# ambicuity/Distributed-LLM-Training-and-Inference-System

Hardware: AMD Instinct MI355X
Metric: tokens/sec (node) GPT-7B train (higher is better)
Workload: dtype bf16; 1 GPU; model=gpt-7b, global_batch=16, seq_len=2048, parallelism=dp1, micro_batch=16, grad_accum=1, activation_checkpoint=none, layout=planner

## Files before the change

llmctl/config/knobs.py:

```python

from __future__ import annotations

import contextlib
import dataclasses
import os
from dataclasses import dataclass, fields
from typing import Any, Dict, Iterator, Optional

ENV = "LLMCTL_KNOBS"


@dataclass(frozen=True)
class PerfKnobs:
    gemm64: bool = True
    gemm64_config: int = 304
    fwd64: str = "auto"
    dgrad64: str = "fused"
    wgrad_kernel: bool = True
    swiglu_bwd: str = "side"
    dgrad_transpose: bool = True
    wt_side_stream: bool = True
    fused_fwd: bool = False
    rope_inplace: bool = True
    fused_rope_attn: bool = True
    moe_pad: bool = True
    overlap_optimizer: bool = False
    gemm_tuning: bool = True
    fa_split: int = -1
    fa_prio: int = 1
    fa_nw: int = 4
    dkv: int = 2
    dkv_nwg: int = 0
    async_tp: bool = True
    async_tp_save_full: bool = False
    cp_zigzag: bool = True
    decode_fused: bool = True
    decode_splits: int = 0
    decode_v3: int = 1
    skinny_gemm: str = "auto"
    prefill_swiglu: bool = True
    prefill_fa: bool = True
    prefill_norm_fold: bool = True
    mixed_steps: bool = True
    custom_ar: bool = True
    tp_graphs: bool = True
    async_decode: bool = True
    tp_fused_decode: bool = True

    def as_dict(self) -> Dict[str, Any]:
        return dataclasses.asdict(self)


NATIVE = ("fa_split", "fa_prio", "fa_nw", "dkv", "dkv_nwg", "decode_splits", "decode_v3")
_FIELDS = {f.name: f for f in fields(PerfKnobs)}


def _coerce(name: str, value: Any) -> Any:
    if name not in _FIELDS:
        raise KeyError(f"unknown performance knob {name!r} (known: {', '.join(sorted(_FIELDS))})")
    typ = _FIELDS[name].type
    if typ in ("bool", bool):
        if isinstance(value, str):
            v = value.strip().lower()
            if v not in ("1", "0", "true", "false", "on", "off", "yes", "no"):
                raise ValueError(f"knob {name}: expected a boolean, got {value!r}")
            return v in ("1", "true", "on", "yes")
        return bool(value)
    if typ in ("int", int):
        return int(value)
    return str(value)


def parse_env(spec: Optional[str]) -> Dict[str, Any]:
    out: Dict[str, Any] = {}
    for part in (spec or "").split(","):
        part = part.strip()
        if not part:
            continue
        if "=" not in part:
            raise ValueError(f"{ENV}: expected name=value, got {part!r}")
        k, v = part.split("=", 1)
        out[k.strip()] = _coerce(k.strip(), v.strip())
    return out


_RETIRED_ENV = ("LLMCTL_SIDE_DGRAD", "LLMCTL_DECODE_ATTN_QKV", "LLMCTL_GEMM64_CONFIG", "LLMCTL_SKINNY")
_warned: set = set()


def _warn_retired_env() -> None:
    import warnings

    names = [f"LLMCTL_{n.upper()}" for n in _FIELDS] + list(_RETIRED_ENV)
    for n in names:
        if n in os.environ and n not in _warned:
            _warned.add(n)
            warnings.warn(f"{n} is no longer read (performance switches are knobs now): set "
                          f"{ENV}=\"{n[7:].lower()}=<value>\" or the [perf] config table instead", stacklevel=3)


def resolve(overrides: Optional[Dict[str, Any]] = None, env: bool = True) -> PerfKnobs:
    _warn_retired_env()
    kw = {k: _coerce(k, v) for k, v in (overrides or {}).items()}
    if env:
        kw.update(parse_env(os.environ.get(ENV)))
    return PerfKnobs(**kw)


_ACTIVE: PerfKnobs = resolve()


def knobs() -> PerfKnobs:
    return _ACTIVE


def push_native(k: Optional[PerfKnobs] = None) -> bool:
    k = k or _ACTIVE
    try:
        from llmctl.ops import _lib

        if not _lib.loaded():
            return False
        import torch

        for name in NATIVE:
            torch.ops.llmctl.set_knob(name, int(getattr(k, name)))
        return True
    except Exception:
        return False


def apply(k: PerfKnobs) -> PerfKnobs:
    global _ACTIVE
    _ACTIVE = k
    push_native(k)
    return k


def use(k: PerfKnobs) -> PerfKnobs:
    if k is not _ACTIVE:
        apply(k)
    return k


def with_env(k: PerfKnobs) -> PerfKnobs:
    env = parse_env(os.environ.get(ENV))
    return dataclasses.replace(k, **env) if env else k


def configure(overrides: Optional[Dict[str, Any]] = None) -> PerfKnobs:
    return apply(resolve(overrides))


@contextlib.contextmanager
def override(**kw: Any) -> Iterator[PerfKnobs]:
    old = _ACTIVE
    new = dataclasses.replace(old, **{k: _coerce(k, v) for k, v in kw.items()})
    apply(new)
    try:
        yield new
    finally:
        apply(old)
```

llmctl/ops/csrc/flash_attn_bwd.hip:

```cpp
#include <cstdlib>
#include <map>
#include <mutex>

#include "attn_common.h"

namespace llmctl {
using namespace attn;
namespace {

constexpr float LOG2E = 1.4426950408889634f;
constexpr int KV_KB = 128;
constexpr int KV_QT = 64;
#ifndef LLMCTL_DKV_NBUF
#define LLMCTL_DKV_NBUF 2
#endif
constexpr int KV_NBUF = LLMCTL_DKV_NBUF;
static_assert(KV_NBUF >= 2 && KV_NBUF <= 4, "dK/dV ring depth 2-4");
constexpr int DQ_QB = 128;
constexpr int DQ_KB = 64;

struct BwdArgs {
  const unsigned short *q, *k, *v, *dout;
  const float* lse;
  const float* delta;
// ... 701 lines not shown
  const int nkb = a.S / KV_KB;
  const int BH = a.B * a.Hkv;
  const bool per_xcd = BH % 8 == 0;
  const int xq = per_xcd ? (int)(blockIdx.x & 7) : 0;
  const int n_items = (per_xcd ? BH / 8 : BH) * nkb;
  const int bh_base = per_xcd ? xq * (BH / 8) : 0;
  const int group = a.Hq / a.Hkv;
  auto pop = [&]() __attribute__((always_inline)) -> int {
    const int j = __hip_atomic_fetch_add(wq + xq, 1, __ATOMIC_RELAXED, __HIP_MEMORY_SCOPE_AGENT);
    return j < n_items ? j : -1;
  };
  if (tid == 0) {
    const int i0 = pop();
    item_w[1] = i0;
    item_w[2] = i0 >= 0 ? pop() : -1;
  }
  __syncthreads();
  int cur = __builtin_amdgcn_readfirstlane(item_w[1]);
  int nxt = __builtin_amdgcn_readfirstlane(item_w[2]);
  if (cur < 0) return;

  const unsigned lds0 = lds_addr(smem);
  unsigned vq[NP], vd[NP];
#pragma unroll
  for (int i = 0; i < NP; ++i) {
    const int byte = (i * 4 + wave) * 1024 + lane * 16;
    const int row = byte / ROWB;
    const int lch = ((byte % ROWB) >> 4) ^ swz_tr<HD>(row);
    vq[i] = (unsigned)((row * a.q_ss + lch * 8) * 2);
    vd[i] = (unsigned)((row * a.do_ss + lch * 8) * 2);
  }
  const float* rc_src = a.rck_w + (wave == 1 ? a.rc_n : 0);
  const unsigned rc_off =
      (unsigned)((32 * (lane >> 5) + 8 * ((lane >> 2) & 3) + 4 * ((lane >> 4) & 1) + (lane & 3)) * 4);

  int iss = cur, iq0 = 0, iq_start = 0, ig = 0;
  const unsigned short *qh = nullptr, *dh = nullptr;
  const float* rh = nullptr;
  bool look_pending = false;
  int n_switch = 0;
  int pend0 = -1, pend1 = -1, npend = 0;
  auto iss_begin = [&](int item) __attribute__((always_inline)) {
    const int bh = bh_base + item / nkb, kb = item % nkb;
    const int bb = bh / a.Hkv, hkk = bh % a.Hkv;
    iq_start = kb * KV_KB;
    iq0 = iq_start;
    ig = 0;
    qh = a.q + bb * a.q_sb + (long)(hkk * group) * a.q_sh;
    dh = a.dout + bb * a.do_sb + (long)(hkk * group) * a.do_sh;
    rh = rc_src + ((long)bb * a.Hq + hkk * group) * a.S;
  };
  iss_begin(cur);
  auto issue = [&](auto slot_c) __attribute__((always_inline)) {
    constexpr int SLC = decltype(slot_c)::value;
    i32x4_t rq = buf_rsrc(qh + (long)iq0 * a.q_ss, (unsigned)(((KV_QT - 1) * a.q_ss + HD) * 2));
    i32x4_t rd = buf_rsrc(dh + (long)iq0 * a.do_ss, (unsigned)(((KV_QT - 1) * a.do_ss + HD) * 2));
    i32x4_t rr = buf_rsrc(rh + iq0, (unsigned)(KV_QT * 4));
    asm volatile("s_nop 4" : "+s"(rq), "+s"(rd), "+s"(rr));
    const unsigned slot = lds0 + (unsigned)(SLC * BUF_B);
#pragma unroll
    for (int i = 0; i < NP; ++i) {
      buf_dma16(rq, vq[i], slot + (i * 4 + wave) * 1024);
      buf_dma16(rd, vd[i], slot + TILE_B + (i * 4 + wave) * 1024);
    }
    buf_dma4(rr, rc_off, slot + 2 * TILE_B + wave * RC_B);
    iq0 += KV_QT;
    if (iq0 >= a.S) {
      if (++ig < group) {
        iq0 = iq_start;
        qh += a.q_sh;
        dh += a.do_sh;
        rh += a.S;
      } else {
        iss = nxt;
        if (iss >= 0) {
          iss_begin(iss);
          if (tid == 0) item_w[3 + (n_switch & 1)] = pop();
          look_pending = true;
          ++n_switch;
        }
        if (npend == 0) pend0 = iss;
        else pend1 = iss;
        ++npend;
      }
    }
  };

  bf16x8_t kf[NKS], vf[NKS];
  auto load_kv = [&](int item) __attribute__((always_inline)) {
    const int bh = bh_base + item / nkb, kb = item % nkb;
    const int bb = bh / a.Hkv, hkk = bh % a.Hkv;
    const int key = kb * KV_KB + wave * 32 + r;
    const unsigned short* Kp = a.k + bb * a.k_sb + hkk * a.k_sh + (long)key * a.k_ss + 8 * hh;
    const unsigned short* Vp = a.v + bb * a.v_sb + hkk * a.v_sh + (long)key * a.v_ss + 8 * hh;
#pragma unroll
    for (int ks = 0; ks < NKS; ++ks) {
      asm volatile("global_load_dwordx4 %0, %1, off" : "+a"(kf[ks]) : "v"(Kp + 16 * ks) : "memory");
      asm volatile("global_load_dwordx4 %0, %1, off" : "+a"(vf[ks]) : "v"(Vp + 16 * ks) : "memory");
    }
  };

  issue(std::integral_constant<int, 0>{});
  load_kv(cur);
  asm volatile("s_waitcnt vmcnt(0)"
               : "+a"(kf[0]), "+a"(kf[1]), "+a"(kf[2]), "+a"(kf[3]), "+a"(kf[4]), "+a"(kf[5]), "+a"(kf[6]),
                 "+a"(kf[7]), "+a"(vf[0]), "+a"(vf[1]), "+a"(vf[2]), "+a"(vf[3]), "+a"(vf[4]), "+a"(vf[5]),
                 "+a"(vf[6]), "+a"(vf[7])
               :
               : "memory");
  __builtin_amdgcn_s_barrier();
  issue(std::integral_constant<int, 1>{});
  f32x16 dk[NDB], dv[NDB];
#pragma unroll
  for (int d = 0; d < NDB; ++d) {
    const bf16x8_t z = {};
    asm volatile("s_nop 2\n\tv_mfma_f32_32x32x16_bf16 %0, %1, %1, 0" : "=a"(dk[d]) : "v"(z));
    asm volatile("v_mfma_f32_32x32x16_bf16 %0, %1, %1, 0" : "=a"(dv[d]) : "v"(z));
  }
  const float c = a.scale_log2;

  int n_done = 0;
  auto stamp = [&](int k) __attribute__((always_inline)) {
    if constexpr (STAMP) {
      if (tid == 0 && n_done < 64)
        a.stamps[(blockIdx.x * 64 + n_done) * 4 + k] = k == 3 ? (unsigned long long)cur : __builtin_amdgcn_s_memrealtime();
    }
  };
  for (;;) {
    stamp(0);
    stamp(3);
    const int bh = bh_base + cur / nkb, kb = cur % nkb;
    const int b = bh / a.Hkv, hk = bh % a.Hkv;
    const int k0 = kb * KV_KB;
    const int wkey0 = k0 + wave * 32;
    const int my_key = wkey0 + r;
    const int ntiles = group * ((a.S - k0) / KV_QT);
    int q0 = k0;
    auto apply_mask = [&](f32x16& s, int h) __attribute__((always_inline)) {
#pragma unroll
      for (int gq = 0; gq < 4; ++gq) {
        const int row0 = q0 + 32 * h + 8 * gq + 4 * hh;
#pragma unroll
        for (int j = 0; j < 4; ++j) s[4 * gq + j] = my_key <= row0 + j ? s[4 * gq + j] : -INFINITY;
      }
    };
    auto tile = [&](auto slot_c) __attribute__((always_inline)) {
      constexpr int SL = decltype(slot_c)::value;
      const bool live = !(wkey0 > q0 + KV_QT - 1);
      if (!live) return;
      const unsigned char* Qs = smem + SL * BUF_B;
      const unsigned char* Ds = Qs + TILE_B;
      const float* lse_s = reinterpret_cast<const float*>(Ds + TILE_B);
      const float* del_s = lse_s + KV_QT;
      const bool need_mask = wkey0 + 31 > q0;
      f32x16 s0 = *reinterpret_cast<const f32x16*>(lse_s + 16 * hh);
      f32x16 p0 = *reinterpret_cast<const f32x16*>(del_s + 16 * hh);
      bf16x8_t qa[NKS], da[NKS];
#pragma unroll
      for (int ks = 0; ks < NKS; ++ks) {
        qa[ks] = lds_read_b128(Qs, tr_off<HD>(r, 2 * ks + hh));
        da[ks] = lds_read_b128(Ds, tr_off<HD>(r, 2 * ks + hh));
      }
      f32x16 s1 = *reinterpret_cast<const f32x16*>(lse_s + 32 + 16 * hh);
      f32x16 p1 = *reinterpret_cast<const f32x16*>(del_s + 32 + 16 * hh);
      bf16x8_t qb[NKS], db[NKS];
#pragma unroll
      for (int ks = 0; ks < NKS; ++ks) {
        mfma_v(s0, qa[ks], kf[ks]);
        qb[ks] = lds_read_b128(Qs, tr_off<HD>(32 + r, 2 * ks + hh));
        mfma_v(p0, da[ks], vf[ks]);
        db[ks] = lds_read_b128(Ds, tr_off<HD>(32 + r, 2 * ks + hh));
      }
      if (need_mask) apply_mask(s0, 0);
      unsigned pw0[8], dw0[8];
      bf16x8_t td[2][NDB], tq[2][NDB];
#pragma unroll
      for (int ks = 0; ks < NKS; ++ks) {
        x_step(s1, p1, qb[ks], kf[ks], db[ks], vf[ks], s0[2 * ks], s0[2 * ks + 1], p0[2 * ks], p0[2 * ks + 1], c,
               pw0[ks], dw0[ks]);
        const int st = ks >> 2, d = ks & 3;
        td[st][d] = tr_frag<HD>(Ds, 16 * st, d * 32, lane);
        tq[st][d] = tr_frag<HD>(Qs, 16 * st, d * 32, lane);
      }
      if (need_mask) apply_mask(s1, 1);
      unsigned pw1[8], dw1[8];
      bf16x8_t cd[2][NDB], cq[2][NDB];
#pragma unroll
      for (int st = 0; st < 2; ++st) {
        const bf16x8_t pb = words8(pw0[4 * st], pw0[4 * st + 1], pw0[4 * st + 2], pw0[4 * st + 3]);
        const bf16x8_t sb = words8(dw0[4 * st], dw0[4 * st + 1], dw0[4 * st + 2], dw0[4 * st + 3]);
#pragma unroll
        for (int d = 0; d < NDB; ++d) {
          const int i = 4 * st + d;
          y_step(dv[d], dk[d], td[st][d], tq[st][d], pb, sb, s1[2 * i], s1[2 * i + 1], p1[2 * i], p1[2 * i + 1], c,
                 pw1[i], dw1[i]);
          cd[st][d] = tr_frag<HD>(Ds, 32 + 16 * st, d * 32, lane);
          cq[st][d] = tr_frag<HD>(Qs, 32 + 16 * st, d * 32, lane);
        }
      }
#pragma unroll
      for (int st = 0; st < 2; ++st) {
        const bf16x8_t pb = words8(pw1[4 * st], pw1[4 * st + 1], pw1[4 * st + 2], pw1[4 * st + 3]);
        const bf16x8_t sb = words8(dw1[4 * st], dw1[4 * st + 1], dw1[4 * st + 2], dw1[4 * st + 3]);
#pragma unroll
        for (int d = 0; d < NDB; ++d) z_step(dv[d], dk[d], cd[st][d], cq[st][d], pb, sb);
      }
    };
    auto advance = [&](auto slot_c) __attribute__((always_inline)) {
      constexpr int SL = decltype(slot_c)::value;
      asm volatile("s_waitcnt lgkmcnt(0)" ::: "memory");
      vm_wait_n<0>();
      __builtin_amdgcn_s_barrier();
      if (look_pending) {
        nxt = __builtin_amdgcn_readfirstlane(item_w[3 + ((n_switch - 1) & 1)]);
        look_pending = false;
      }
      if (iss >= 0) issue(std::integral_constant<int, SL>{});
      q0 += KV_QT;
      if (q0 >= a.S) q0 = k0;
    };
    for (int t = 0; t < ntiles; t += 2) {
      tile(std::integral_constant<int, 0>{});
      advance(std::integral_constant<int, 0>{});
      tile(std::integral_constant<int, 1>{});
      advance(std::integral_constant<int, 1>{});
    }
    stamp(1);
    {
      const long tok = (long)b * a.S + my_key;
      unsigned short* dkp = a.dk + tok * a.dk_st + (long)hk * HD;
      unsigned short* dvp = a.dv + tok * a.dv_st + (long)hk * HD;
      const bool rope = a.cos_t != nullptr;
      f32x4 cs[NDB / 2][4], sn[NDB / 2][4];
      if (rope) {
        const long p = a.rope_pos ? (long)a.rope_pos[tok] : tok % a.rope_S;
        const float* cr = a.cos_t + p * (HD / 2);
        const float* sr = a.sin_t + p * (HD / 2);
#pragma unroll
        for (int d = 0; d < NDB / 2; ++d)
#pragma unroll
          for (int g = 0; g < 4; ++g) {
            const int col = d * 32 + 8 * g + 4 * hh;
            cs[d][g] = *reinterpret_cast<const f32x4*>(cr + col);
            sn[d][g] = *reinterpret_cast<const f32x4*>(sr + col);
          }
      }
#pragma unroll
      for (int d = 0; d < NDB; ++d) asm volatile("s_nop 7\n\ts_nop 7" : "+a"(dk[d]), "+a"(dv[d]));
      auto st8 = [&](unsigned short* p, const float* x, float mul) __attribute__((always_inline)) {
        s2_t w;
        w[0] = (unsigned)f2bf(x[0] * mul) | ((unsigned)f2bf(x[1] * mul) << 16);
        w[1] = (unsigned)f2bf(x[2] * mul) | ((unsigned)f2bf(x[3] * mul) << 16);
        asm volatile("global_store_dwordx2 %0, %1, off" ::"v"(p), "v"(w) : "memory");
      };
#pragma unroll
      for (int d = 0; d < NDB / 2; ++d) {
        const f32x16 x1 = acc_copy(dk[d]), x2 = acc_copy(dk[d + NDB / 2]);
        acc_zero(dk[d]);
        acc_zero(dk[d + NDB / 2]);
#pragma unroll
        for (int g = 0; g < 4; ++g) {
          const int col = d * 32 + 8 * g + 4 * hh;
          float lo[4], hi[4];
#pragma unroll
          for (int j = 0; j < 4; ++j) {
            const float c1 = rope ? cs[d][g][j] : 1.f, s1 = rope ? sn[d][g][j] : 0.f;
            lo[j] = x1[4 * g + j] * c1 + x2[4 * g + j] * s1;
            hi[j] = x2[4 * g + j] * c1 - x1[4 * g + j] * s1;
          }
          st8(dkp + col, lo, a.scale);
          st8(dkp + col + HD / 2, hi, a.scale);
        }
      }
#pragma unroll
      for (int d = 0; d < NDB; ++d) {
        const f32x16 x = acc_copy(dv[d]);
        acc_zero(dv[d]);
#pragma unroll
        for (int g = 0; g < 4; ++g) {
          float y[4];
#pragma unroll
          for (int j = 0; j < 4; ++j) y[j] = x[4 * g + j];
          st8(dvp + d * 32 + 8 * g + 4 * hh, y, 1.f);
        }
      }
      load_kv(pend0 >= 0 ? pend0 : cur);
      asm volatile("s_waitcnt vmcnt(0)"
                   : "+a"(kf[0]), "+a"(kf[1]), "+a"(kf[2]), "+a"(kf[3]), "+a"(kf[4]), "+a"(kf[5]), "+a"(kf[6]),
                     "+a"(kf[7]), "+a"(vf[0]), "+a"(vf[1]), "+a"(vf[2]), "+a"(vf[3]), "+a"(vf[4]), "+a"(vf[5]),
                     "+a"(vf[6]), "+a"(vf[7])
                   :
                   : "memory");
    }
    stamp(2);
    ++n_done;
    if (pend0 < 0) break;
    cur = pend0;
    pend0 = pend1;
    pend1 = -1;
    --npend;
  }
}

template <int HD, bool CAUSAL, bool DOC>
__global__ __launch_bounds__(256, 2) void fa_bwd_dq_kernel(BwdArgs a) {
  constexpr int NKS = HD / 16;
  constexpr int NDB = HD / 32;
  constexpr int ROWB = HD * 2;
  constexpr int TILE = DQ_KB * ROWB;
  constexpr int PPW = TILE / 1024 / 4;
  constexpr int SLOT = 2 * TILE;
  __shared__ __attribute__((aligned(1024))) unsigned char smem[2 * SLOT];

  const int tid = threadIdx.x;
  const int lane = tid & 63;
  const int wave = __builtin_amdgcn_readfirstlane(tid >> 6);
  const int r = lane & 31, hh = lane >> 5;
  const int nqb = (a.S + DQ_QB - 1) / DQ_QB;
  const int BH = a.B * a.Hq;
  int bh, qi;
  if (BH % 8) {
    bh = blockIdx.x % BH;
    qi = blockIdx.x / BH;
  } else {
    const int x = blockIdx.x & 7, j = blockIdx.x >> 3;
    bh = x * (BH >> 3) + j / nqb;
    qi = j % nqb;
  }
  const int qblk = nqb - 1 - qi;
  const int b = bh / a.Hq, hq = bh % a.Hq;
  const int hk = hq / (a.Hq / a.Hkv);
  const int q_row0 = qblk * DQ_QB + wave * 32;
  const int my_q = q_row0 + r;
  const int qc = min(my_q, a.S - 1);

  const unsigned short* Kp = a.k + b * a.k_sb + hk * a.k_sh;
  const unsigned short* Vp = a.v + b * a.v_sb + hk * a.v_sh;

#pragma unroll
  for (int i = 0; i < 2 * SLOT / 4096; ++i)
    *reinterpret_cast<uint4*>(smem + i * 4096 + tid * 16) = make_uint4(0, 0, 0, 0);

  bf16x8_t qf[NKS], df[NKS];
  {
    const unsigned short* Qp = a.q + b * a.q_sb + hq * a.q_sh + (long)qc * a.q_ss + 8 * hh;
    const unsigned short* Dp = a.dout + b * a.do_sb + hq * a.do_sh + (long)qc * a.do_ss + 8 * hh;
#pragma unroll
    for (int ks = 0; ks < NKS; ++ks) {
      qf[ks] = __builtin_bit_cast(bf16x8_t, gload16(Qp + 16 * ks));
      df[ks] = __builtin_bit_cast(bf16x8_t, gload16(Dp + 16 * ks));
    }
  }
  const long rc = ((long)b * a.Hq + hq) * a.S + qc;
  const float nlse2 = -a.lse[rc] * LOG2E;
  float dlt;
  if (a.o != nullptr) {
    const unsigned short* Op = a.o + b * a.o_sb + hq * a.o_sh + (long)qc * a.o_ss + 8 * hh;
    float acc = 0.f;
#pragma unroll
    for (int ks = 0; ks < NKS; ++ks) {
      const bf16x8_t of = __builtin_bit_cast(bf16x8_t, gload16(Op + 16 * ks));
#pragma unroll
      for (int j = 0; j < 8; ++j) acc += (float)of[j] * (float)df[ks][j];
    }
    dlt = xor32_add(acc);
    if (hh == 0 && my_q < a.S) a.delta_w[rc] = dlt;
  } else {
    dlt = a.delta[rc];
  }
  if (hh == 0 && my_q < a.S) {
    a.rck_w[rc] = -a.lse[rc] / a.scale;
    a.rck_w[a.rc_n + rc] = -dlt;
  }
#pragma unroll
  for (int ks = 0; ks < NKS; ++ks) asm volatile("" ::"v"(qf[ks]), "v"(df[ks]));
  asm volatile("" ::"v"(nlse2), "v"(dlt));

  f32x16 dq[NDB];
#pragma unroll
  for (int d = 0; d < NDB; ++d)
#pragma unroll
    for (int i = 0; i < 16; ++i) dq[d][i] = 0.f;

  const int kv_end = CAUSAL ? min(a.S, qblk * DQ_QB + DQ_QB) : a.S;
  const int ntiles = (kv_end + DQ_KB - 1) / DQ_KB;
  int my_start = 0, w_min = 0, w_max = 0, t0 = 0;
  if constexpr (DOC) {
    const int* ds = a.doc + (long)b * a.S;
    my_start = ds[qc];
    w_min = __builtin_amdgcn_readfirstlane(ds[min(q_row0, a.S - 1)]);
    w_max = __builtin_amdgcn_readfirstlane(ds[min(q_row0 + 31, a.S - 1)]);
    t0 = __builtin_amdgcn_readfirstlane(ds[min(qblk * DQ_QB, a.S - 1)]) / DQ_KB;
  }
  const int key_hi = CAUSAL ? qc : a.S - 1;
  int klo[NDB], khi[NDB];
#pragma unroll
  for (int d = 0; d < NDB; ++d) tr_frag_offs<HD>(d * 32, lane, klo[d], khi[d]);
  int kro[NKS], vro[NKS];
#pragma unroll
  for (int ks = 0; ks < NKS; ++ks) {
    kro[ks] = tr_off<HD>(r, 2 * ks + hh);
    vro[ks] = row_off<HD>(r, 2 * ks + hh);
  }

  unsigned vk[PPW], vv[PPW];
#pragma unroll
  for (int i = 0; i < PPW; ++i) {
    const int byte = (i * 4 + wave) * 1024 + lane * 16;
    const int row = byte / ROWB, pch = (byte % ROWB) >> 4;
    vk[i] = (unsigned)((row * a.k_ss + ((pch ^ swz_tr<HD>(row)) << 3)) * 2);
    vv[i] = (unsigned)((row * a.v_ss + ((pch ^ swz_row<HD>(row)) << 3)) * 2);
  }
  const unsigned lds0 = lds_addr(smem);
  int ik0 = t0 * DQ_KB;
  const unsigned short* kc = Kp + (long)ik0 * a.k_ss;
  const unsigned short* vc = Vp + (long)ik0 * a.v_ss;
  const long k_step = (long)DQ_KB * a.k_ss, v_step = (long)DQ_KB * a.v_ss;
  auto issue = [&](auto slot_c) __attribute__((always_inline)) {
    constexpr int SLC = decltype(slot_c)::value;
    const int nk = min(DQ_KB, a.S - ik0);
    i32x4_t rk = buf_rsrc(kc, (unsigned)(((nk - 1) * a.k_ss + HD) * 2));
    i32x4_t rv = buf_rsrc(vc, (unsigned)(((nk - 1) * a.v_ss + HD) * 2));
    asm volatile("s_nop 4" : "+s"(rk), "+s"(rv));
    const unsigned slot = lds0 + (unsigned)(SLC * SLOT) + wave * 1024;
#pragma unroll
    for (int i = 0; i < PPW; ++i) {
      buf_dma16(rk, vk[i], slot + i * 4096);
      buf_dma16(rv, vv[i], slot + TILE + i * 4096);
    }
    ik0 += DQ_KB;
    kc += k_step;
    vc += v_step;
  };

  auto tile = [&](bool need_mask, const unsigned char* Ks, const unsigned char* Vs, int kv0)
                  __attribute__((always_inline)) {
#pragma unroll
    for (int kb = 0; kb < 2; ++kb) {
      f32x16 s, dp;
#pragma unroll
      for (int i = 0; i < 16; ++i) s[i] = dp[i] = 0.f;
#pragma unroll
      for (int ks = 0; ks < NKS; ++ks) {
        s = mfma32(lds_read_b128(Ks, kb * 32 * (HD * 2) + kro[ks]), qf[ks], s);
        dp = mfma32(lds_read_b128(Vs, kb * 32 * (HD * 2) + vro[ks]), df[ks], dp);
      }
      if (need_mask) {
#pragma unroll
        for (int i = 0; i < 16; ++i) {
          const int key = kv0 + kb * 32 + acc_row(i, hh);
          bool ok = key <= key_hi;
          if constexpr (DOC) ok = ok && key >= my_start;
          s[i] = ok ? s[i] : -INFINITY;
        }
      }
      float dsv[16];
#pragma unroll
      for (int i = 0; i < 16; ++i) dsv[i] = fast_exp2(__builtin_fmaf(s[i], a.scale_log2, nlse2)) * (dp[i] - dlt);
#pragma unroll
      for (int st = 0; st < 2; ++st) {
        const bf16x8_t sbf = to_bf16x8(dsv + 8 * st);
#pragma unroll
        for (int d = 0; d < NDB; ++d) dq[d] = mfma32(tr_frag_at<HD>(Ks, kb * 32 + 16 * st, klo[d], khi[d]), sbf, dq[d]);
      }
    }
  };

  __syncthreads();
  auto step = [&](auto slot_c, int t) __attribute__((always_inline)) {
    constexpr int SL = decltype(slot_c)::value;
    vm_wait_n<0>();
    __builtin_amdgcn_s_barrier();
    if (t + 1 < ntiles) issue(std::integral_constant<int, 1 - SL>{});
    const int kv0 = t * DQ_KB;
    bool live = true;
    if constexpr (CAUSAL) live = kv0 <= q_row0 + 31;
    if constexpr (DOC) live = live && kv0 + DQ_KB > w_min;
    if (live) {
      const bool need_mask =
          (CAUSAL && kv0 + DQ_KB - 1 > q_row0) || (kv0 + DQ_KB > a.S) || (DOC && kv0 < w_max);
      tile(need_mask, smem + SL * SLOT, smem + SL * SLOT + TILE, kv0);
    }
  };
  if (t0 < ntiles) issue(std::integral_constant<int, 0>{});
  for (int t = t0; t < ntiles; t += 2) {
    step(std::integral_constant<int, 0>{}, t);
    if (t + 1 < ntiles) step(std::integral_constant<int, 1>{}, t + 1);
  }
  if (my_q < a.S) {
    const long tok = (long)b * a.S + my_q;
    const float *cr = nullptr, *sr = nullptr;
    if (a.cos_t != nullptr) {
      const long p = a.rope_pos ? (long)a.rope_pos[tok] : tok % a.rope_S;
      cr = a.cos_t + p * (HD / 2);
      sr = a.sin_t + p * (HD / 2);
    }
    store_row<HD>(a.dq + tok * a.dq_st + (long)hq * HD, dq, a.scale, hh, cr, sr);
  }
}

int dkv_mode() {
  const int64_t m = knob("dkv", 2);
  return (m >= 0 && m <= 2) ? (int)m : 2;
}

int* dkv_queue(hipStream_t s) {
  static std::mutex mu;
  static std::map<std::pair<int, hipStream_t>, int*> bufs;
  int dev = 0;
  LLMCTL_HIP_CHECK(hipGetDevice(&dev));
  std::lock_guard<std::mutex> lk(mu);
  int*& q = bufs[{dev, s}];
  if (q == nullptr) LLMCTL_HIP_CHECK(hipMalloc(&q, 64 * sizeof(int)));
  return q;
}

template <int HD, bool CAUSAL, bool DOC>
void launch_bwd(const BwdArgs& a, hipStream_t s, bool do_dq, bool do_dkv, int dkv_impl) {
  if (do_dq) {
    const int nqb = (a.S + DQ_QB - 1) / DQ_QB;
    hipLaunchKernelGGL((fa_bwd_dq_kernel<HD, CAUSAL, DOC>), dim3((unsigned)(a.B * a.Hq * nqb)), dim3(256), 0, s, a);
  }
  if (do_dkv) {
    const int nkb = (a.S + KV_KB - 1) / KV_KB;
    const dim3 grid((unsigned)(a.B * a.Hkv * nkb));
    if constexpr (HD == 128 && CAUSAL) {
      if (dkv_impl == 2 && a.stamps != nullptr) {
        hipLaunchKernelGGL((fa_bwd_dkv_pipe_kernel<HD, CAUSAL, DOC, true>), grid, dim3(256), 0, s, a);
        return;
      }
      if constexpr (!DOC) {
        if (a.S % KV_KB == 0 && (dkv_impl == 3 || dkv_impl == 4 || (dkv_impl < 0 && dkv_mode() == 2))) {
          int* wq = dkv_queue(s);
          LLMCTL_HIP_CHECK(hipMemsetAsync(wq, 0, 8 * sizeof(int), s));
          int nwg = std::min<long>((long)num_cus(), (long)a.B * a.Hkv * nkb);
          const int min_wg = ((long)a.B * a.Hkv) % 8 == 0 ? 8 : 1;
          if (const int64_t e = knob("dkv_nwg", 0); e > 0) nwg = std::max<int>(min_wg, std::min<int>(nwg, (int)e));
          nwg = std::max(nwg, min_wg);
          if (a.stamps != nullptr)
            hipLaunchKernelGGL(fa_bwd_dkv_persist_kernel<true>, dim3((unsigned)nwg), dim3(256), 0, s, a, wq);
          else
            hipLaunchKernelGGL(fa_bwd_dkv_persist_kernel<false>, dim3((unsigned)nwg), dim3(256), 0, s, a, wq);
          return;
        }
      }
      if (dkv_impl == 1 || dkv_impl == 3 || (dkv_impl < 0 && dkv_mode() >= 1)) {
        hipLaunchKernelGGL((fa_bwd_dkv_pipe_kernel<HD, CAUSAL, DOC>), grid, dim3(256), 0, s, a);
        return;
      }
    }
    hipLaunchKernelGGL((fa_bwd_dkv_kernel<HD, CAUSAL, DOC>), grid, dim3(256), 0, s, a);
  }
}

void dispatch_bwd(const BwdArgs& a, int D, bool causal, bool doc, hipStream_t s, bool do_dq = true,
                  bool do_dkv = true, int dkv_impl = -1) {
  if (doc) {
    if (D == 128) launch_bwd<128, true, true>(a, s, do_dq, do_dkv, dkv_impl);
    else launch_bwd<64, true, true>(a, s, do_dq, do_dkv, dkv_impl);
  } else if (D == 128) {
    if (causal) launch_bwd<128, true, false>(a, s, do_dq, do_dkv, dkv_impl);
    else launch_bwd<128, false, false>(a, s, do_dq, do_dkv, dkv_impl);
  } else {
    if (causal) launch_bwd<64, true, false>(a, s, do_dq, do_dkv, dkv_impl);
    else launch_bwd<64, false, false>(a, s, do_dq, do_dkv, dkv_impl);
  }
}

BwdArgs make_args(const at::Tensor& dout, const at::Tensor& q, const at::Tensor& k, const at::Tensor& v,
                  const at::Tensor& lse, const at::Tensor& delta, at::Tensor& dq, at::Tensor& dk, at::Tensor& dv,
                  double scale) {
  return BwdArgs{bf_ptr(q), bf_ptr(k), bf_ptr(v), bf_ptr(dout), lse.data_ptr<float>(), delta.data_ptr<float>(),
                 bf_mut(dq), bf_mut(dk), bf_mut(dv), (int)q.size(0), (int)q.size(1), (int)q.size(2),
                 (int)k.size(2), q.stride(0), q.stride(1), q.stride(2), k.stride(0), k.stride(1), k.stride(2),
                 v.stride(0), v.stride(1), v.stride(2), dout.stride(0), dout.stride(1), dout.stride(2),
                 (float)scale, (float)(scale * 1.4426950408889634), nullptr,
                 (long)dq.size(2) * dq.size(3), (long)dk.size(2) * dk.size(3), (long)dv.size(2) * dv.size(3),
                 nullptr, nullptr, nullptr, 0, nullptr, 0, 0, 0, nullptr, nullptr, 0};
}

at::Tensor row_consts(BwdArgs& a, const at::Tensor& lse) {
  auto rck = at::empty({2 * lse.numel()}, lse.options());
  a.rck_w = rck.data_ptr<float>();
  a.rc_n = lse.numel();
  return rck;
}

}

std::tuple<at::Tensor, at::Tensor, at::Tensor> flash_attn_bwd(const at::Tensor& dout, const at::Tensor& q,
                                                              const at::Tensor& k, const at::Tensor& v,
                                                              const at::Tensor& o, const at::Tensor& lse,
                                                              double scale, bool causal,
                                                              const c10::optional<at::Tensor>& doc_start) {
  LLMCTL_CHECK(q.dim() == 4 && k.dim() == 4 && v.dim() == 4 && o.dim() == 4 && dout.dim() == 4,
               "flash_attn_bwd: [B,S,H,D] tensors");
  const int B = q.size(0), S = q.size(1), Hq = q.size(2), D = q.size(3);
  const int Hkv = k.size(2);
  LLMCTL_CHECK(D == 64 || D == 128, "head_dim must be 64 or 128");
  LLMCTL_CHECK(Hkv > 0 && Hq % Hkv == 0, "Hq must be a multiple of Hkv");
  LLMCTL_CHECK(dout.sizes() == q.sizes() && o.sizes() == q.sizes() && k.sizes() == v.sizes() && k.size(0) == B &&
                   k.size(1) == S && k.size(3) == D,
               "shape mismatch");
  LLMCTL_CHECK(lse.scalar_type() == at::kFloat && lse.is_contiguous() && lse.numel() == (long)B * Hq * S,
               "lse must be contiguous fp32 [B,Hq,S]");
  for (const at::Tensor* t : {&dout, &q, &k, &v, &o})
    LLMCTL_CHECK(t->is_cuda() && t->scalar_type() == at::kBFloat16 && t->stride(3) == 1 && t->stride(0) % 8 == 0 &&
                     t->stride(1) % 8 == 0 && t->stride(2) % 8 == 0 &&
                     (reinterpret_cast<uintptr_t>(t->data_ptr()) & 15) == 0,
                 "flash_attn_bwd: bf16, d-contiguous, 16-B aligned rows");
  const c10::DeviceGuard g(q.device());
  auto delta = at::empty({B, Hq, S}, q.options().dtype(at::kFloat));
  auto dq = at::empty({B, S, Hq, D}, q.options());
  auto dk = at::empty({B, S, Hkv, D}, q.options());
  auto dv = at::empty({B, S, Hkv, D}, q.options());
  if ((long)B * S * Hq == 0) return {dq, dk, dv};
  auto s = stream();
  BwdArgs a = make_args(dout, q, k, v, lse, delta, dq, dk, dv, scale);
  a.o = bf_ptr(o);
  a.o_sb = o.stride(0);
  a.o_ss = o.stride(1);
  a.o_sh = o.stride(2);
  a.delta_w = delta.data_ptr<float>();
  auto rck = row_consts(a, lse);
  bool doc = false;
  if (doc_start.has_value() && doc_start->defined()) {
    const at::Tensor& ds = *doc_start;
    LLMCTL_CHECK(causal && ds.is_cuda() && ds.scalar_type() == at::kInt && ds.is_contiguous() && ds.dim() == 2 &&
                     ds.size(0) == B && ds.size(1) == S,
                 "flash_attn_bwd: doc_start must be contiguous int32 [B,S] (causal)");
    a.doc = ds.data_ptr<int>();
    doc = true;
  }
  dispatch_bwd(a, D, causal, doc, s);
  return {dq, dk, dv};
}

at::Tensor flash_attn_bwd_qkv(const at::Tensor& dout, const at::Tensor& q, const at::Tensor& k, const at::Tensor& v,
                              const at::Tensor& o, const at::Tensor& lse, double scale, bool causal,
                              const c10::optional<at::Tensor>& doc_start, const at::Tensor& cos_t,
                              const at::Tensor& sin_t, const c10::optional<at::Tensor>& positions, int64_t seq_len) {
  LLMCTL_CHECK(q.dim() == 4 && k.dim() == 4 && v.dim() == 4 && o.dim() == 4 && dout.dim() == 4,
               "flash_attn_bwd_qkv: [B,S,H,D] tensors");
  const int B = q.size(0), S = q.size(1), Hq = q.size(2), D = q.size(3);
  const int Hkv = k.size(2);
  LLMCTL_CHECK(D == 64 || D == 128, "head_dim must be 64 or 128");
  LLMCTL_CHECK(Hkv > 0 && Hq % Hkv == 0, "Hq must be a multiple of Hkv");
  LLMCTL_CHECK(dout.sizes() == q.sizes() && o.sizes() == q.sizes() && k.sizes() == v.sizes() && k.size(0) == B &&
                   k.size(1) == S && k.size(3) == D,
               "shape mismatch");
  LLMCTL_CHECK(lse.scalar_type() == at::kFloat && lse.is_contiguous() && lse.numel() == (long)B * Hq * S,
               "lse must be contiguous fp32 [B,Hq,S]");
  for (const at::Tensor* t : {&dout, &q, &k, &v, &o})
    LLMCTL_CHECK(t->is_cuda() && t->scalar_type() == at::kBFloat16 && t->stride(3) == 1 && t->stride(0) % 8 == 0 &&
                     t->stride(1) % 8 == 0 && t->stride(2) % 8 == 0 &&
                     (reinterpret_cast<uintptr_t>(t->data_ptr()) & 15) == 0,
                 "flash_attn_bwd_qkv: bf16, d-contiguous, 16-B aligned rows");
  LLMCTL_CHECK(cos_t.is_cuda() && sin_t.is_cuda() && cos_t.scalar_type() == at::kFloat &&
                   sin_t.scalar_type() == at::kFloat && cos_t.is_contiguous() && sin_t.is_contiguous() &&
                   cos_t.dim() == 2 && cos_t.size(1) == D / 2 && sin_t.sizes() == cos_t.sizes(),
               "flash_attn_bwd_qkv: cos/sin fp32 contiguous [P, D/2]");
  const bool has_pos = positions.has_value() && positions->defined();
  if (has_pos) {
    LLMCTL_CHECK(positions->is_cuda() && positions->scalar_type() == at::kInt && positions->is_contiguous() &&
                     positions->numel() == (long)B * S,
                 "flash_attn_bwd_qkv: positions int32 [B*S]");
  } else {
    LLMCTL_CHECK(seq_len > 0 && seq_len <= cos_t.size(0), "flash_attn_bwd_qkv: seq_len within the tables");
  }
  const c10::DeviceGuard g(q.device());
  const long W = (long)(Hq + 2 * Hkv) * D;
  auto dqkv = at::empty({(long)B * S, W}, q.options());
  if ((long)B * S * Hq == 0) return dqkv;
  auto delta = at::empty({B, Hq, S}, q.options().dtype(at::kFloat));
  auto s = stream();
  unsigned short* base = bf_mut(dqkv);
  BwdArgs a{bf_ptr(q), bf_ptr(k), bf_ptr(v), bf_ptr(dout), lse.data_ptr<float>(), delta.data_ptr<float>(),
            base, base + (long)Hq * D, base + (long)(Hq + Hkv) * D, B, S, Hq, Hkv,
            q.stride(0), q.stride(1), q.stride(2), k.stride(0), k.stride(1), k.stride(2),
            v.stride(0), v.stride(1), v.stride(2), dout.stride(0), dout.stride(1), dout.stride(2),
            (float)scale, (float)(scale * 1.4426950408889634), nullptr, W, W, W,
            cos_t.data_ptr<float>(), sin_t.data_ptr<float>(), has_pos ? positions->data_ptr<int>() : nullptr,
            (int)(has_pos ? 1 : seq_len), bf_ptr(o), o.stride(0), o.stride(1), o.stride(2),
            delta.data_ptr<float>(), nullptr, 0};
  auto rck = row_consts(a, lse);
  bool doc = false;
  if (doc_start.has_value() && doc_start->defined()) {
    const at::Tensor& ds = *doc_start;
    LLMCTL_CHECK(causal && ds.is_cuda() && ds.scalar_type() == at::kInt && ds.is_contiguous() && ds.dim() == 2 &&
                     ds.size(0) == B && ds.size(1) == S,
                 "flash_attn_bwd_qkv: doc_start must be contiguous int32 [B,S] (causal)");
    a.doc = ds.data_ptr<int>();
    doc = true;
  }
  dispatch_bwd(a, D, causal, doc, s);
  return dqkv;
}

void fa_bwd_ablate(const at::Tensor& dout, const at::Tensor& q, const at::Tensor& k, const at::Tensor& v,
                   const at::Tensor& delta, const at::Tensor& lse, at::Tensor& dq, at::Tensor& dk, at::Tensor& dv,
                   int64_t abl) {
  const int D = q.size(3);
  LLMCTL_CHECK(D == 64 || D == 128, "fa_bwd_ablate: head_dim 64 or 128");
  LLMCTL_CHECK(dq.scalar_type() == at::kBFloat16 && dq.sizes() == q.sizes() && dk.sizes() == k.sizes() &&
                   dv.sizes() == k.sizes() && delta.numel() == lse.numel(),
               "fa_bwd_ablate: bf16 dq/dk/dv, fp32 delta");
  const c10::DeviceGuard g(q.device());
  const double scale = 1.0 / std::sqrt((double)D);
  BwdArgs a = make_args(dout, q, k, v, lse, delta, dq, dk, dv, scale);
  if (abl == 5 || abl == 7) {
    LLMCTL_CHECK(dq.numel() * 2 >= (long)q.size(0) * k.size(2) * ((q.size(1) + KV_KB - 1) / KV_KB) * 64,
                 "fa_bwd_ablate: dq too small for the timeline");
    a.stamps = reinterpret_cast<unsigned long long*>(dq.data_ptr());
  }
  auto rck = row_consts(a, lse);
  if (abl == 1 || abl >= 3) {
    rck.narrow(0, 0, lse.numel()).copy_(lse.reshape(-1) * (-1.0 / scale));
    rck.narrow(0, lse.numel(), lse.numel()).copy_(-delta.reshape(-1));
  }
  dispatch_bwd(a, D, true, false, stream(), abl == 0 || abl == 2, abl != 2, abl >= 3 ? (int)abl - 3 : -1);
}

TORCH_LIBRARY_IMPL(llmctl, CUDA, m) {
  m.impl("flash_attn_bwd", &flash_attn_bwd);
  m.impl("flash_attn_bwd_qkv", &flash_attn_bwd_qkv);
  m.impl("fa_bwd_ablate", &fa_bwd_ablate);
}

}
```

Before: 30170 tokens/s.

## Software-pipeline LDS reads with MFMAs in flash-attention dQ backward kernel

Adds a pipelined tile path to the dQ backward kernel. It prefetches K/V fragments from LDS four MFMAs ahead, overlaps the transposed-K reads and the dS exponent computation with the dQ MFMAs, and preloads the next sub-block's fragments, with sched_barriers fixing the order. The aim is to hide LDS latency behind matrix-core work. It is controlled by a new native knob dq_pipe, default on. It costs more registers and a second template instantiation, and the fixed schedule may hurt occupancy.

```diff
diff --git a/llmctl/config/knobs.py b/llmctl/config/knobs.py
--- a/llmctl/config/knobs.py
+++ b/llmctl/config/knobs.py
@@ -29,6 +29,7 @@
     fa_split: int = -1
     fa_prio: int = 1
     fa_nw: int = 4
+    dq_pipe: int = 1
     dkv: int = 2
     dkv_nwg: int = 0
     async_tp: bool = True
@@ -51,7 +52,7 @@
         return dataclasses.asdict(self)
 
 
-NATIVE = ("fa_split", "fa_prio", "fa_nw", "dkv", "dkv_nwg", "decode_splits", "decode_v3")
+NATIVE = ("fa_split", "fa_prio", "fa_nw", "dq_pipe", "dkv", "dkv_nwg", "decode_splits", "decode_v3")
 _FIELDS = {f.name: f for f in fields(PerfKnobs)}
 
 
diff --git a/llmctl/ops/csrc/flash_attn_bwd.hip b/llmctl/ops/csrc/flash_attn_bwd.hip
--- a/llmctl/ops/csrc/flash_attn_bwd.hip
+++ b/llmctl/ops/csrc/flash_attn_bwd.hip
@@ -1027,7 +1027,7 @@
   }
 }
 
-template <int HD, bool CAUSAL, bool DOC>
+template <int HD, bool CAUSAL, bool DOC, int PIPE>
 __global__ __launch_bounds__(256, 2) void fa_bwd_dq_kernel(BwdArgs a) {
   constexpr int NKS = HD / 16;
   constexpr int NDB = HD / 32;
@@ -1158,8 +1158,78 @@
     vc += v_step;
   };
 
+  auto tile_pipe = [&](bool need_mask, const unsigned char* Ks, const unsigned char* Vs, int kv0)
+                       __attribute__((always_inline)) {
+    constexpr int NS = 2 * NKS, NQ = 2 * NDB, EPG = 8 / NDB;
+    bf16x8_t fr[4], tf[3];
+    auto rd = [&](int kb, int n) __attribute__((always_inline)) {
+      return lds_read_b128((n & 1) ? Vs : Ks, kb * 32 * (HD * 2) + ((n & 1) ? vro[n / 2] : kro[n / 2]));
+    };
+    auto rd_t = [&](int kb, int m) __attribute__((always_inline)) {
+      return tr_frag_at<HD>(Ks, kb * 32 + (m / NDB) * 16, klo[m % NDB], khi[m % NDB]);
+    };
+    auto ds1 = [&](float sv, float dpv) __attribute__((always_inline)) {
+      return fast_exp2(__builtin_fmaf(sv, a.scale_log2, nlse2)) * (dpv - dlt);
+    };
+#pragma unroll
+    for (int n = 0; n < 4; ++n) fr[n] = rd(0, n);
+    __builtin_amdgcn_sched_barrier(0);
+#pragma unroll
+    for (int kb = 0; kb < 2; ++kb) {
+      f32x16 s, dp;
+#pragma unroll
+      for (int i = 0; i < 16; ++i) s[i] = dp[i] = 0.f;
+#pragma unroll
+      for (int g = 0; g < NS; ++g) {
+        if (g & 1) dp = mfma32(fr[g % 4], df[g / 2], dp);
+        else s = mfma32(fr[g % 4], qf[g / 2], s);
+        if (g + 4 < NS) fr[g % 4] = rd(kb, g + 4);
+        if (g + 3 >= NS) tf[g + 3 - NS] = rd_t(kb, g + 3 - NS);
+        __builtin_amdgcn_sched_barrier(0);
+      }
+      if (need_mask) {
+#pragma unroll
+        for (int i = 0; i < 16; ++i) {
+          const int key = kv0 + kb * 32 + acc_row(i, hh);
+          bool ok = key <= key_hi;
+          if constexpr (DOC) ok = ok && key >= my_start;
+          s[i] = ok ? s[i] : -INFINITY;
+        }
+      }
+      float dsv[16];
+#pragma unroll
+      for (int i = 0; i < 8; ++i) dsv[i] = ds1(s[i], dp[i]);
+      bf16x8_t sbf = to_bf16x8(dsv);
+      __builtin_amdgcn_sched_barrier(0);
+#pragma unroll
+      for (int m = 0; m < NQ; ++m) {
+        dq[m % NDB] = mfma32(tf[m % 3], sbf, dq[m % NDB]);
+        if (m + 3 < NQ) tf[m % 3] = rd_t(kb, m + 3);
+        if (m < NDB) {
+#pragma unroll
+          for (int e = 8 + m * EPG; e < 8 + (m + 1) * EPG; ++e) dsv[e] = ds1(s[e], dp[e]);
+        } else if (kb == 0) {
+          if (m - NDB < 4) fr[m - NDB] = rd(1, m - NDB);
+          if (NDB < 4 && m == NQ - 1) {
+#pragma unroll
+            for (int n = NDB; n < 4; ++n) fr[n] = rd(1, n);
+          }
+        }
+        __builtin_amdgcn_sched_barrier(0);
+        if (m == NDB - 1) {
+          sbf = to_bf16x8(dsv + 8);
+          __builtin_amdgcn_sched_barrier(0);
+        }
+      }
+    }
+  };
+
   auto tile = [&](bool need_mask, const unsigned char* Ks, const unsigned char* Vs, int kv0)
                   __attribute__((always_inline)) {
+    if constexpr (PIPE) {
+      tile_pipe(need_mask, Ks, Vs, kv0);
+      return;
+    }
 #pragma unroll
     for (int kb = 0; kb < 2; ++kb) {
       f32x16 s, dp;
@@ -1244,7 +1314,9 @@
 void launch_bwd(const BwdArgs& a, hipStream_t s, bool do_dq, bool do_dkv, int dkv_impl) {
   if (do_dq) {
     const int nqb = (a.S + DQ_QB - 1) / DQ_QB;
-    hipLaunchKernelGGL((fa_bwd_dq_kernel<HD, CAUSAL, DOC>), dim3((unsigned)(a.B * a.Hq * nqb)), dim3(256), 0, s, a);
+    const dim3 grid((unsigned)(a.B * a.Hq * nqb));
+    if (knob("dq_pipe", 1) != 0) hipLaunchKernelGGL((fa_bwd_dq_kernel<HD, CAUSAL, DOC, 1>), grid, dim3(256), 0, s, a);
+    else hipLaunchKernelGGL((fa_bwd_dq_kernel<HD, CAUSAL, DOC, 0>), grid, dim3(256), 0, s, a);
   }
   if (do_dkv) {
     const int nkb = (a.S + KV_KB - 1) / KV_KB;
```

Measured after the change: 30190 tokens/s, median of 6. Within noise of the previous version (+0.0%).
